# SAP/nested-hashing-psi

Measured on AMD Instinct MI355X. Metric: server PIE ciphertexts/sec, higher is better.
Workload: dtype u64

## Files before the change

nested_hashing_psi_amd/csrc/kernels.hpp:

```cpp
#pragma once
#include <hip/hip_runtime.h>

#include <atomic>
#include <vector>

#include "params.hpp"

namespace piehip {

struct PerDeviceOnce {
    std::atomic<unsigned long long> done{0};
    bool first_on_current_device()
    {
        int dev = 0;
        if (hipGetDevice(&dev) != hipSuccess || dev < 0 || dev > 63) return true;
        const unsigned long long bit = 1ULL << dev;
        return (done.fetch_or(bit) & bit) == 0;
    }
};

enum class NttKernel { radix2, blocked32, blocked16 };
struct NttRoute {
    NttKernel kernel;
    u32 s0;
// ... 7 lines not shown
    const u64 *twc = nullptr;
    const u64 *twc_fold = nullptr;
    const u64 *twk16 = nullptr;
    const DevConsts *dc;
    u32 N, logN;
    u32 num_cus;
    u32 max_slots = 0;
    bool lane_order = false;
    bool fold = false;
    NttKernel lane_kernel = NttKernel::radix2;
    u32 lane_logn = 0;
    u32 lane_T = 0;
    u32 lane_kp = 16;
    bool small_moduli = false;
    bool fold_moduli = false;
    bool xq_reuse = false;
    bool x_direct = false;
    bool fused_tensor = false;
    bool d01_eval_q = false;
    bool result_eval_q = false;
    bool digits_with_d01 = false;
    bool digit_lift_lane = false;
    bool digit_lift_std = false;
    u32 transform_cus() const
    {
        if (!max_slots) return num_cus;
        const u32 c = (max_slots + 1) / 2;
        return c < num_cus ? (c ? c : 1u) : num_cus;
    }
};
// ... 166 lines not shown
```

nested_hashing_psi_amd/csrc/kernels_ntt16.hip:

```cpp
#include <cassert>

#include "kernels.hpp"
#include "ntt16_kernel.h"

namespace piehip {

void build_twk16_table(const u64 *nat_pairs, u32 s0, u32 slice_log, std::vector<u64> &out)
{
    if (slice_log == 14)
        ntt16::build_twk_table_t<14>(nat_pairs, s0, out);
    else
        ntt16::build_twk_table_t<13>(nat_pairs, s0, out);
}

void ntt16_sigma_inverse_map(u32 logN, u32 s0, std::vector<u32> &map)
{
    const u32 N = 1u << logN, n = N >> s0;
    map.resize(N);
    for (u32 p = 0; p < N; p++) map[p] = (p / n) * n + ntt16::lane_to_std_t(p % n, n / 16);
}

template <u32 LOGNS, auto KERNEL>
static void launch_ntt16_k(const ntt16::Args &a, u32 num_cus, hipStream_t st)
{
    typedef ntt16::Geo<LOGNS> G;
    constexpr size_t lds = (size_t)G::LDS_WORDS * sizeof(u64);
    static PerDeviceOnce attr;
    if (attr.first_on_current_device()) (void)hipFuncSetAttribute((const void *)KERNEL, hipFuncAttributeMaxDynamicSharedMemorySize, (int)lds);
    const u32 slots = (LOGNS == 13 ? 2u : 1u) * num_cus;
    const u32 grid = a.nitems < slots ? a.nitems : slots;
    hipLaunchKernelGGL(KERNEL, dim3(grid), dim3(G::T), lds, st, a);
}
template <u32 LOGNS>
static void launch_ntt16_t(const ntt16::Args &a, bool inverse, bool lift, u32 num_cus, hipStream_t st, bool tensor = false, bool fd = false)
{
    using ntt16::ntt16_kernel_t;
    if (tensor && fd) launch_ntt16_k<LOGNS, ntt16_kernel_t<LOGNS, true, false, true, ArithKind::fold>>(a, num_cus, st);
    else if (tensor) launch_ntt16_k<LOGNS, ntt16_kernel_t<LOGNS, true, false, true>>(a, num_cus, st);
    else if (inverse) launch_ntt16_k<LOGNS, ntt16_kernel_t<LOGNS, true>>(a, num_cus, st);
    else if (lift) launch_ntt16_k<LOGNS, ntt16_kernel_t<LOGNS, false, true>>(a, num_cus, st);
    else launch_ntt16_k<LOGNS, ntt16_kernel_t<LOGNS, false>>(a, num_cus, st);
}

void launch_ntt16(const NttPlan &pl, u64 *data, u32 nlimbs, u32 mod_base, u32 mod_count, bool inverse, bool sigma, hipStream_t st,
                  const NttExtra *ex, const Ntt16Digits *dg)
{
    const bool folded = pl.fold;
    const u32 s0 = folded ? 1u : 0u;
    assert(ntt_route(pl, inverse, sigma, folded).kernel == NttKernel::blocked16 && (!dg || pl.digits_with_d01));
    ntt16::Args a;
    a.data = data;
    a.twp = reinterpret_cast<const ntt16::u64x2 *>(pl.twp);
    a.twk = reinterpret_cast<const ntt16::u64x2 *>(pl.twk16);
    a.dc = pl.dc;
    a.N = pl.N;
    a.s0 = s0;
    a.nitems = nlimbs << s0;
// ... 15 lines not shown
    a.lift_src = nullptr;
    a.lift_stride = 0;
    a.lift_L = 1;
    a.tsrc = nullptr;
    a.tq_L = 0;
    a.tq_first = 0;
    if (dg && !inverse) {
        a.lift_first = a.nitems;
        a.nitems += (dg->nb * dg->L * dg->L) << s0;
        a.data2 = dg->dig;
        a.lift_src = dg->d2;
        a.lift_stride = dg->stride2;
        a.lift_L = dg->L;
    }
    const bool lift = a.lift_first != ~0u;
    if (pl.lane_logn == 14)
        launch_ntt16_t<14>(a, inverse, lift, pl.transform_cus(), st);
    else
        launch_ntt16_t<13>(a, inverse, lift, pl.transform_cus(), st);
}

void launch_ntt16_tensor(const NttPlan &pl, const u64 *e, u64 *d, u32 nb, u32 M, hipStream_t st, u32 eval_q_L, bool eval_q_d2)
{
    assert(pl.fused_tensor && (!eval_q_L || ((eval_q_d2 ? pl.result_eval_q : pl.d01_eval_q) && eval_q_L < M)) && (!eval_q_d2 || eval_q_L));
    const bool folded = pl.fold;
    const u32 s0 = folded ? 1u : 0u;
    ntt16::Args a = {};
    a.data = d;
    a.twp = reinterpret_cast<const ntt16::u64x2 *>(pl.twp);
    a.twk = reinterpret_cast<const ntt16::u64x2 *>(pl.twk16);
    a.dc = pl.dc;
    a.N = pl.N;
    a.s0 = s0;
    a.tq_L = eval_q_L;
// ... 17 lines not shown
```

nested_hashing_psi_amd/csrc/ntt16_bfly.inc:

```
#define NTT16_CT1(TWC) \
    asm( \
        "v_mad_u64_u32 v[120:121], vcc, %[bl0], %[sh0], 0\n\t" \
        "v_lshl_add_u64 v[118:119], %[a0], 0, %[nq4]\n\t" \
        "v_mad_u64_u32 v[120:121], vcc, %[bh0], %[sl0], v[120:121]\n\t" \
        "v_mad_u64_u32 v[124:125], vcc, %[bl0], %[wl0], 0\n\t" \
        "v_lshlrev_b32 v117, 1, %[bh0]\n\t" \
        "v_ashrrev_i32 v122, 31, v119\n\t" \
        "v_bfi_b32 v118, v122, %[al0], v118\n\t" \
        "v_bfi_b32 v119, v122, %[ah0], v119\n\t" \
        "v_mad_u64_u32 v[126:127], vcc, %[bl0], %[wh0], 0\n\t" \
        "v_lshrrev_b64 v[120:121], 31, v[120:121]\n\t" \
        "v_mad_u64_u32 v[126:127], vcc, %[bh0], %[wl0], v[126:127]\n\t" \
        "v_mad_u64_u32 v[122:123], vcc, v117, %[sh0], v[120:121]\n\t" \
        "v_mad_u64_u32 v[124:125], vcc, v122, %[nql], v[124:125]\n\t" \
        "v_mad_u64_u32 v[126:127], vcc, v122, %[nqh], v[126:127]\n\t" \
        "v_mad_u64_u32 v[126:127], vcc, v123, %[nql], v[126:127]\n\t" \
        "v_lshl_add_u64 v[122:123], v[118:119], 0, %[q4]\n\t" \
        "v_sub_co_u32 %[bol0], vcc, v122, v124\n\t" \
        "v_add_u32 v125, v125, v126\n\t" \
        "v_lshl_add_u64 %[ao0], v[118:119], 0, v[124:125]\n\t" \
        "v_subb_co_u32 %[boh0], vcc, v123, v125, vcc\n\t" \
        : [ao0] "=v"(ao0), [bol0] "=v"(bol0), [boh0] "=v"(boh0) \
        : [a0] "v"(a0), [al0] "v"((u32)a0), [ah0] "v"((u32)(a0 >> 32)), [bl0] "v"((u32)b0), [bh0] "v"((u32)(b0 >> 32)), \
          [wl0] TWC(t0.wl), [wh0] TWC(t0.wh), [sl0] TWC(t0.sl), [sh0] TWC(t0.sh), \
// ... 120 lines not shown
        "v_mad_u64_u32 v[126:127], vcc, %[bh0], %[wl0], v[126:127]\n\t" \
        "v_mad_u64_u32 v[124:125], vcc, %[bh0], %[sh20], v[122:123]\n\t" \
        "v_mad_u64_u32 %[a0], vcc, v124, %[nql], %[a0]\n\t" \
        "v_mad_u64_u32 v[126:127], vcc, v124, %[nqh], v[126:127]\n\t" \
        "v_lshl_add_u64 v[120:121], v[120:121], 1, %[q4]\n\t" \
        "v_sub_co_u32 %[bol0], vcc, v120, %[al0]\n\t" \
        "v_mad_u64_u32 v[126:127], %[cs], v125, %[nql], v[126:127]\n\t" \
        "v_add_u32 %[ah0], %[ah0], v126\n\t" \
        "v_subb_co_u32 %[boh0], vcc, v121, %[ah0], vcc\n\t" \
        : [a0] "+v"(a0), [bol0] "=v"(bol0), [boh0] "=v"(boh0), [cs] "=s"(cs) \
        : [al0] "v"((u32)a0), [ah0] "v"((u32)(a0 >> 32)), [bl0] "v"((u32)b0), [bh0] "v"((u32)(b0 >> 32)), \
          [wl0] TWC(t0.wl), [wh0] TWC(t0.wh), [sl0] TWC(t0.sl), [sh0] TWC(t0.sh), \
          [sh20] TWC(t0.sh2), \
          [nql] "s"(m.nql), [nqh] "s"(m.nqh), [nq4] "s"(m.nq4), [q4] "s"(m.q4) \
        : "vcc", "v119", "v120", "v121", "v122", "v123", "v124", "v125", "v126", "v127")
```

nested_hashing_psi_amd/csrc/ntt16_kernel.h:

```cpp
#pragma once
#include <vector>

#include "madasm.h"
#include "params.hpp"

namespace piehip {
namespace ntt16 {

typedef u64 u64x2 __attribute__((ext_vector_type(2)));

template <u32 LOGNS>
struct Geo {
    static constexpr u32 LOGN = LOGNS;
    static constexpr u32 NS = 1u << LOGNS;
    static constexpr u32 T = NS / 16;
    static constexpr u32 W = T / 64;
    static constexpr u32 R = NS / 1024;
    static constexpr u32 LOGR = LOGNS - 10;
    static constexpr u32 CPT = 16 / R;
    static constexpr u32 LDS_WORDS = NS + NS / 16;
    static constexpr u32 TWK_PER_SLICE = W * 15 * 16 + W * 12 * 64;
};
static constexpr u32 LOGN = Geo<13>::LOGN, NS = Geo<13>::NS, T = Geo<13>::T, LDS_WORDS = Geo<13>::LDS_WORDS,
                     TWK_PER_SLICE = Geo<13>::TWK_PER_SLICE;
// ... 15 lines not shown
    u32 nql, nqh;
    u64 nq4;
    u64 q4;
};

#ifndef NTT16_CT_SEEDED
#define NTT16_CT_SEEDED 1
#endif
#define NTT16_S(x) "s"(x)
#define NTT16_V(x) "v"(x)
#include "ntt16_bfly.inc"

#ifndef NTT16_INV_H2
#define NTT16_INV_H2 1
#endif
template <bool INV, bool SC, bool H2 = SC && (!INV || NTT16_INV_H2)>
__device__ __forceinline__ void bfly(u64 &x0, u64 &y0, const Tw &t0, const ModC &m)
{
    u64 a0 = x0;
    const u64 b0 = y0;
    if (INV) {
        u32 aol0, aoh0;
        u64 bo0;
        if (SC && H2)
            NTT16_GS1H(NTT16_S);
        else if (SC)
            NTT16_GS1(NTT16_S);
        else if (H2)
            NTT16_GS1H(NTT16_V);
        else
            NTT16_GS1(NTT16_V);
        x0 = ((u64)aoh0 << 32) | aol0, y0 = bo0;
    } else {
        u32 bol0, boh0;
#if NTT16_CT_SEEDED
        u64 cs;
// ... 9 lines not shown
        x0 = a0, y0 = ((u64)boh0 << 32) | bol0;
#else
        u64 ao0;
        if (SC && H2)
            NTT16_CT1H(NTT16_S);
        else if (SC)
            NTT16_CT1(NTT16_S);
        else if (H2)
            NTT16_CT1H(NTT16_V);
        else
            NTT16_CT1(NTT16_V);
        x0 = ao0, y0 = ((u64)boh0 << 32) | bol0;
#endif
    }
}
template <bool INV, bool SC, bool H2 = SC && !INV>
__device__ __forceinline__ void bfly2(u64 &x0, u64 &y0, const Tw &t0, u64 &x1, u64 &y1, const Tw &t1, const ModC &m)
{
    bfly<INV, SC, H2>(x0, y0, t0, m);
    bfly<INV, SC, H2>(x1, y1, t1, m);
}
__device__ __forceinline__ constexpr int bfly_lo(int m, int d) { return ((m & ~(d - 1)) << 1) | (m & (d - 1)); }

typedef const __attribute__((address_space(4))) u64x2 *TwS;
typedef const __attribute__((address_space(4))) DevConsts *DcS;
__device__ __forceinline__ u64 uniform_addr(const void *p)
{
    const u64 v = (u64)p;
    const u32 lo = __builtin_amdgcn_readfirstlane((u32)v), hi = __builtin_amdgcn_readfirstlane((u32)(v >> 32));
    return ((u64)hi << 32) | lo;
}

__device__ __forceinline__ u64 csub_neg(u64 x, u64 negm)
{
    u32 lo, hi;
    asm("v_lshl_add_u64 v[126:127], %[x], 0, %[nm]\n\t"
        "v_ashrrev_i32 v125, 31, v127\n\t"
        "v_bfi_b32 %[lo], v125, %[xl], v126\n\t"
        "v_bfi_b32 %[hi], v125, %[xh], v127"
        : [lo] "=&v"(lo), [hi] "=&v"(hi)
        : [x] "v"(x), [xl] "v"((u32)x), [xh] "v"((u32)(x >> 32)), [nm] "s"(negm)
        : "v125", "v126", "v127");
    return ((u64)hi << 32) | lo;
}

__device__ __forceinline__ const u64 *at_bytes(const u64 *ubase, u32 boff)
{
    return reinterpret_cast<const u64 *>(reinterpret_cast<const char *>(ubase) + boff);
}
__device__ __forceinline__ u64 *at_bytes(u64 *ubase, u32 boff) { return reinterpret_cast<u64 *>(reinterpret_cast<char *>(ubase) + boff); }
__device__ __forceinline__ const u64x2 *at_bytes(const u64x2 *ubase, u32 boff)
{
    return reinterpret_cast<const u64x2 *>(reinterpret_cast<const char *>(ubase) + boff);
}

template <u32 CPT>
__device__ __forceinline__ void row_get(u64 *x, int r, const u64 *p)
// ... 241 lines not shown
                const u64 fc = csub2_neg(k ? vc[j].y : vc[j].x, nq4, nq2);
                const u64 fd = csub2_neg(k ? vd[j].y : vd[j].x, nq4, nq2);
                colacc_mac(c, split30(fc), split30(fd));
            }
            x[2 * j + k] = FD ? colacc_fold_to_4q(c.c0, c.c1, c.c2, nq) : colacc123_to_4q(c.c0, c.c1, c.c2, mu, nq);
        }
        NTT16_FENCE();
        if (j + DEPTH < 8) NTT16_TLOAD(j + DEPTH);
    }
#undef NTT16_TLOAD
}

template <u32 LOGNS, bool INV, bool LIFT = false, bool TENSOR = false, ArithKind KIND = ArithKind::barrett>
__global__ void __launch_bounds__(Geo<LOGNS>::T, 4) ntt16_kernel_t(Args a)
{
    static_assert(KIND == ArithKind::barrett || (TENSOR && KIND == ArithKind::fold), "the kind: of the tensor load phase, column accumulators");
    constexpr bool FD = KIND == ArithKind::fold;
    typedef Geo<LOGNS> G;
    constexpr u32 NS = G::NS, T = G::T, R = G::R, LOGR = G::LOGR, CPT = G::CPT, TWK_PER_SLICE = G::TWK_PER_SLICE;
    extern __shared__ __attribute__((aligned(16))) u64 lds[];
    const u32 tau = threadIdx.x;
    const u32 w = __builtin_amdgcn_readfirstlane(tau >> 6), l = tau & 63;
    const u32 la = l >> 2, lc = l & 3;
    u64 *const p1 = lds + phi(CPT * tau);
    u64 *const p2 = lds + phi(1024 * w + l);
    u64 *const p3 = lds + 1088 * w + 68 * la + lc;
    u64 *const p4 = lds + phi(1024 * w + 16 * l);

    u64 x[16];
    auto limb_of = [&](u32 it) -> u32 {
        u32 lb = it >> a.s0;
        if (!INV && a.skip_L) {
// ... 87 lines not shown
                };
                if (a.s0 == 1) {
                    u64x2 fw;
                    fw.x = dcs->fold_w[lj];
                    fw.y = dcs->fold_w_sh[lj] >> 1;
                    const Tw t = make_tw(fw);
                    u64 y[16];
#pragma unroll
                    for (int r = 0; r < (int)R; r++) {
                        row_get_global<CPT>(x, r, at_bytes(src + 1024 * r, coffb));
                        row_get_global<CPT>(y, r, at_bytes(src + NS + 1024 * r, coffb));
                    }
#pragma unroll
                    for (int k = 0; k < 16; k++) {
                        u64 u0 = lift1(x[k]), v0 = lift1(y[k]);
                        bfly<false, true>(u0, v0, t, mc);
                        x[k] = blk ? v0 : u0;
                    }
                } else {
#pragma unroll
                    for (int r = 0; r < (int)R; r++) row_get_global<CPT>(x, r, at_bytes(src + 1024 * r, coffb));
#pragma unroll
                    for (int k = 0; k < 16; k++) x[k] = lift1(x[k]);
                }
            } else {
#pragma unroll
                for (int r = 0; r < (int)R; r++) row_get_global<CPT>(x, r, at_bytes(g + 1024 * r, coffb));
            }
            NTT16_PRIO_F(1);
#pragma unroll
            for (int s = 0; s < (int)LOGR; s++) {
                const int d = (int)(R >> 1) >> s;
#pragma unroll
                for (int r = 0; r < (int)R; r++) {
                    if (r & d) continue;
                    const Tw t = make_tw(NTT16_TWL(1u << s, (u32)r >> (LOGR - s)));
#pragma unroll
                    for (int c = 0; c < (int)CPT; c++) bfly<false, true>(x[CPT * r + c], x[CPT * (r + d) + c], t, mc);
                }
            }
            NTT16_STAMP(1);
            __syncthreads();
            NTT16_STAMP(2);
#pragma unroll
            for (int r = 0; r < (int)R; r++) row_put<CPT>(x, r, p1 + 1088 * r);
            NTT16_STAMP(3);
            __syncthreads();
            NTT16_STAMP(4);
            NTT16_PRIO_F(2);
#pragma unroll
            for (int k = 0; k < 16; k++) x[k] = p2[68 * k];
#pragma unroll
            for (int sb = 0; sb < 4; sb++) {
                const int d = 8 >> sb;
#pragma unroll
                for (int mm = 0; mm < 8; mm += 2) {
                    const int k0 = bfly_lo(mm, d), k1 = bfly_lo(mm + 1, d);
                    const Tw t0 = make_tw(NTT16_TWL(G::W << sb, (w << sb) + ((u32)k0 >> (4 - sb))));
                    const Tw t1 = make_tw(NTT16_TWL(G::W << sb, (w << sb) + ((u32)k1 >> (4 - sb))));
                    bfly2<false, true>(x[k0], x[k0 + d], t0, x[k1], x[k1 + d], t1, mc);
                }
            }
            NTT16_LOAD3(t7, 0);
            NTT16_LOAD3(t8, 1);
#pragma unroll
            for (int k = 0; k < 16; k++) p2[68 * k] = x[k];
            NTT16_STAMP(5);
            wave_sync();
            NTT16_PRIO_F(3);
#pragma unroll
            for (int k = 0; k < 16; k++) x[k] = p3[4 * k + 2 * (k >> 3)];
            NTT16_LOAD3(t9, 2);
            NTT16_FENCE();
            {
                const Tw t = make_tw(t7[0]);
#pragma unroll
                for (int k = 0; k < 8; k += 2) bfly2<false, false, true>(x[k], x[k + 8], t, x[k + 1], x[k + 9], t, mc);
            }
            NTT16_LOAD3H(t10, 3, 0);
            NTT16_FENCE();
#pragma unroll
            for (int mm = 0; mm < 8; mm += 2) {
                const int k0 = bfly_lo(mm, 4), k1 = bfly_lo(mm + 1, 4);
                bfly2<false, false, true>(x[k0], x[k0 + 4], make_tw(t8[k0 >> 3]), x[k1], x[k1 + 4], make_tw(t8[k1 >> 3]), mc);
            }
            NTT16_LOAD3H(t10, 3, 4);
            NTT16_FENCE();
#pragma unroll
            for (int mm = 0; mm < 8; mm += 2) {
                const int k0 = bfly_lo(mm, 2), k1 = bfly_lo(mm + 1, 2);
                bfly2<false, false>(x[k0], x[k0 + 2], make_tw(t9[k0 >> 2]), x[k1], x[k1 + 2], make_tw(t9[k1 >> 2]), mc);
            }
            NTT16_LOAD4(t11, 0, 4);
            NTT16_FENCE();
#pragma unroll
            for (int k = 0; k < 16; k += 4)
                bfly2<false, false>(x[k], x[k + 1], make_tw(t10[k >> 1]), x[k + 2], x[k + 3], make_tw(t10[(k >> 1) + 1]), mc);
#pragma unroll
            for (int k = 0; k < 16; k++) p3[4 * k + 2 * (k >> 3)] = x[k];
            NTT16_STAMP(6);
            wave_sync();
            NTT16_PRIO_F(4);
#pragma unroll
            for (int j = 0; j < 8; j++) {
                const u64x2 v = *reinterpret_cast<const u64x2 *>(p4 + 2 * j);
                x[2 * j] = v.x;
                x[2 * j + 1] = v.y;
            }
            NTT16_LOAD4(t12, 4, 4);
            NTT16_FENCE();
#pragma unroll
            for (int g4 = 0; g4 < 4; g4++) {
                const Tw t = make_tw(t11[g4]);
                bfly2<false, false>(x[4 * g4], x[4 * g4 + 2], t, x[4 * g4 + 1], x[4 * g4 + 3], t, mc);
                if (g4 == 1) {
                    NTT16_FENCE();
                    _Pragma("unroll") for (int j_ = 4; j_ < 8; j_++) t12[j_] = *at_bytes(tw4 + 64 * (4 + j_), lb);
                    NTT16_FENCE();
                }
            }
            NTT16_FENCE();
#pragma unroll
            for (int k = 0; k < 16; k += 4)
                bfly2<false, false>(x[k], x[k + 1], make_tw(t12[k >> 1]), x[k + 2], x[k + 3], make_tw(t12[(k >> 1) + 1]), mc);
            NTT16_STAMP(7);
            const bool lazy = (a.flags & F_LAZY_OUT) != 0 && !lift;
            if (!lazy) {
#pragma unroll
                for (int k = 0; k < 16; k++) x[k] = csub_neg(csub_neg(csub_neg(x[k], 0 - q4), 0 - q2), 0 - q);
            }
#pragma unroll
            for (int j = 0; j < 8; j++) {
                u64x2 v;
                v.x = x[2 * j], v.y = x[2 * j + 1];
                pair_put_global(v, at_bytes(g + 2 * T * j, voffb));
            }
            NTT16_STAMP(8);
        } else {
            NTT16_STAMP(0);
            NTT16_PRIO_I(0);
            NTT16_LOAD4(t12, 4, 4);
            const bool is_x = !TENSOR && (a.flags & F_STD_IN) && a.copy_out && (limb / (2 * a.copy_L)) % a.copy_K == 0;
            u64 *co = nullptr;
            if (is_x) {
// ... 46 lines not shown
                else
                    tensor_load<T, false, FD>(x, pa, pb, pc, pd, voffb, q, mu);
            } else {
                const u64 *src = x_in ? co : g;
                asm("" : "+s"(src));
#pragma unroll
                for (int j = 0; j < 8; j++) {
                    const u64x2 v = pair_get_global(at_bytes(src + 2 * T * j, voffb));
                    x[2 * j] = v.x, x[2 * j + 1] = v.y;
                }
            }
            NTT16_FENCE();
            _Pragma("unroll") for (int j_ = 4; j_ < 8; j_++) t12[j_] = *at_bytes(tw4 + 64 * (4 + j_), lb);
            NTT16_FENCE();
            NTT16_PRIO_I(1);
#pragma unroll
            for (int k = 0; k < 16; k += 4) {
                bfly2<true, false>(x[k], x[k + 1], make_tw(t12[k >> 1]), x[k + 2], x[k + 3], make_tw(t12[(k >> 1) + 1]), mc);
                if (k == 4) {
                    NTT16_FENCE();
                    NTT16_LOAD4(t11, 0, 4);
                    NTT16_FENCE();
                }
            }
            NTT16_LOAD3(t10, 3);
            NTT16_FENCE();
#pragma unroll
            for (int g4 = 0; g4 < 4; g4++) {
                const Tw t = make_tw(t11[g4]);
                bfly2<true, false>(x[4 * g4], x[4 * g4 + 2], t, x[4 * g4 + 1], x[4 * g4 + 3], t, mc);
            }
            NTT16_STAMP(1);
            NTT16_STAMP(2);
#pragma unroll
            for (int j = 0; j < 8; j++) {
                u64x2 v;
                v.x = x[2 * j];
                v.y = x[2 * j + 1];
                *reinterpret_cast<u64x2 *>(p4 + 2 * j) = v;
            }
            wave_sync();
            NTT16_STAMP(3);
            NTT16_PRIO_I(2);
#pragma unroll
            for (int k = 0; k < 16; k++) x[k] = p3[4 * k + 2 * (k >> 3)];
            NTT16_LOAD3(t9, 2);
            NTT16_FENCE();
#pragma unroll
            for (int k = 0; k < 16; k += 4)
                bfly2<true, false>(x[k], x[k + 1], make_tw(t10[k >> 1]), x[k + 2], x[k + 3], make_tw(t10[(k >> 1) + 1]), mc);
            NTT16_LOAD3(t8, 1);
            NTT16_LOAD3(t7, 0);
            NTT16_FENCE();
#pragma unroll
            for (int mm = 0; mm < 8; mm += 2) {
                const int k0 = bfly_lo(mm, 2), k1 = bfly_lo(mm + 1, 2);
                bfly2<true, false>(x[k0], x[k0 + 2], make_tw(t9[k0 >> 2]), x[k1], x[k1 + 2], make_tw(t9[k1 >> 2]), mc);
            }
            NTT16_FENCE();
#pragma unroll
            for (int mm = 0; mm < 8; mm += 2) {
                const int k0 = bfly_lo(mm, 4), k1 = bfly_lo(mm + 1, 4);
                bfly2<true, false>(x[k0], x[k0 + 4], make_tw(t8[k0 >> 3]), x[k1], x[k1 + 4], make_tw(t8[k1 >> 3]), mc);
            }
            {
                const Tw t = make_tw(t7[0]);
#pragma unroll
                for (int k = 0; k < 8; k += 2) bfly2<true, false>(x[k], x[k + 8], t, x[k + 1], x[k + 9], t, mc);
            }
#pragma unroll
            for (int k = 0; k < 16; k++) p3[4 * k + 2 * (k >> 3)] = x[k];
            wave_sync();
            NTT16_STAMP(4);
            NTT16_PRIO_I(3);
#pragma unroll
            for (int k = 0; k < 16; k++) x[k] = p2[68 * k];
#pragma unroll
            for (int sb = 3; sb >= 0; sb--) {
                const int d = 8 >> sb;
#pragma unroll
                for (int mm = 0; mm < 8; mm += 2) {
                    const int k0 = bfly_lo(mm, d), k1 = bfly_lo(mm + 1, d);
                    const Tw t0 = make_tw(NTT16_TWL(G::W << sb, (w << sb) + ((u32)k0 >> (4 - sb))));
                    const Tw t1 = make_tw(NTT16_TWL(G::W << sb, (w << sb) + ((u32)k1 >> (4 - sb))));
                    bfly2<true, true>(x[k0], x[k0 + d], t0, x[k1], x[k1 + d], t1, mc);
                }
            }
#pragma unroll
            for (int k = 0; k < 16; k++) p2[68 * k] = x[k];
            NTT16_STAMP(5);
            __syncthreads();
            NTT16_STAMP(6);
            NTT16_PRIO_I(4);
#pragma unroll
            for (int r = 0; r < (int)R; r++) row_get<CPT>(x, r, p1 + 1088 * r);
            __syncthreads();
#pragma unroll
            for (int s = (int)LOGR - 1; s >= 0; s--) {
                const int d = (int)(R >> 1) >> s;
#pragma unroll
                for (int r = 0; r < (int)R; r++) {
                    if (r & d) continue;
                    const Tw t = make_tw(NTT16_TWL(1u << s, (u32)r >> (LOGR - s)));
#pragma unroll
                    for (int c = 0; c < (int)CPT; c++) bfly<true, true>(x[CPT * r + c], x[CPT * (r + d) + c], t, mc);
                }
            }
            NTT16_STAMP(7);
            const u64 n_inv = dcs->mod[mod].n_inv, n_inv_sh = dcs->mod[mod].n_inv_sh;
            if (!(a.flags & F_FOLDED)) {
#pragma unroll
                for (int k = 0; k < 16; k++) {
                    if (a.s0 == 0)
                        x[k] = csub_neg(mul_shoup_lazy(x[k], n_inv, n_inv_sh, q), 0 - q);
                    else
                        x[k] = csub_neg(csub_neg(x[k], 0 - q2), 0 - q);
                }
            }
#pragma unroll
            for (int r = 0; r < (int)R; r++) row_put_global<CPT>(x, r, at_bytes(g + 1024 * r, coffb));
            NTT16_STAMP(8);
// ... 12 lines not shown
```

nested_hashing_psi_amd/csrc/piehip.cpp:

```cpp
#include "piehip_ctx.hpp"

#include <random>

using namespace piehip;

static thread_local std::string g_err;
static const char *KNAMES[PIEHIP_NKERNELS] = {"stage_a_mac", "ntt_fwd", "ntt_inv",  "expand",   "tensor",    "scale_round",
                                              "digits",      "relin",   "mask_mul", "encode",   "automorph", "other",
                                              "event_pair",  "tensor_ntt_inv", "result_ntt_inv", "limb_drop", "result_ntt_fwd",
                                              "deg2_finish"};
static void free_workspace(piehip_ctx *h);

namespace piehip {

int fail(int code, const std::string &msg)
{
    g_err = msg;
    return code;
}

void join_pending(piehip_ctx *h)
{
    if (!h->pending_join) return;
    for (size_t g = 0; g < h->ev_join.size(); g++) (void)hipStreamWaitEvent(h->stream, h->ev_join[g], 0);
// ... 128 lines not shown
    do {                                                                               \
        hipError_t e_ = (expr);                                                        \
        if (e_ != hipSuccess) return std::string(#expr) + ": " + hipGetErrorString(e_); \
    } while (0)
    const u32 N = hp.N, M = hp.M, logN = hp.logN;
    pl.N = N;
    pl.logN = logN;
    {
        bool lazy_ok = true, small_moduli = true, fold_moduli = true;
        for (u32 a = 0; a <= M; a++) {
            if (hp.moduli[a] >> 60) lazy_ok = false;
            if (a < M && (hp.moduli[a] >> 59) != 1) small_moduli = false;
            if (a < M && (1ull << 60) - hp.moduli[a] >= COLACC_FOLD_MAX_D) fold_moduli = false;
        }
        ntt_plan_decide(pl, lazy_ok, small_moduli, fold_moduli);
        hipDeviceProp_t prop;
        pl.num_cus = (hipGetDeviceProperties(&prop, h->device) == hipSuccess && prop.multiProcessorCount > 0) ? (u32)prop.multiProcessorCount : 256u;
    }
    TBL_(upload_table(h, &hp.dc, 1, d_dc));
    pl.dc = *d_dc;
    {
        std::vector<u64> pairs((size_t)(M + 1) * 4 * N);
        u64 *tables = nullptr;
        TBL_(upload_table(h, (const u64 *)nullptr, pairs.size(), &tables));
        pl.tables = tables;
        for (u32 a = 0; a <= M; a++) {
            for (const std::vector<u64> *t : {&hp.tw[a], &hp.tw_sh[a], &hp.itw[a], &hp.itw_sh[a]}) {
                TBL_(hipMemcpy(tables, t->data(), sizeof(u64) * N, hipMemcpyHostToDevice));
                tables += N;
            }
// ... 1044 lines not shown
```

Baseline: 81200.

## Use fold-reduction butterflies in blocked16 NTT for pseudo-Mersenne moduli

Result: faster. 83500 (median of 6 runs) (+2.8%).

```diff
diff --git a/nested_hashing_psi_amd/csrc/kernels.hpp b/nested_hashing_psi_amd/csrc/kernels.hpp
--- a/nested_hashing_psi_amd/csrc/kernels.hpp
+++ b/nested_hashing_psi_amd/csrc/kernels.hpp
@@ -45,6 +45,7 @@
     u32 lane_kp = 16;
     bool small_moduli = false;
     bool fold_moduli = false;
+    u32 fold_mod_count = 0;
     bool xq_reuse = false;
     bool x_direct = false;
     bool fused_tensor = false;
diff --git a/nested_hashing_psi_amd/csrc/kernels_ntt16.hip b/nested_hashing_psi_amd/csrc/kernels_ntt16.hip
--- a/nested_hashing_psi_amd/csrc/kernels_ntt16.hip
+++ b/nested_hashing_psi_amd/csrc/kernels_ntt16.hip
@@ -31,16 +31,26 @@
     const u32 grid = a.nitems < slots ? a.nitems : slots;
     hipLaunchKernelGGL(KERNEL, dim3(grid), dim3(G::T), lds, st, a);
 }
+template <u32 LOGNS, ArithKind KIND>
+static void launch_ntt16_kind(const ntt16::Args &a, bool inverse, bool lift, u32 num_cus, hipStream_t st, bool tensor)
+{
+    using ntt16::ntt16_kernel_t;
+    if (tensor) launch_ntt16_k<LOGNS, ntt16_kernel_t<LOGNS, true, false, true, KIND>>(a, num_cus, st);
+    else if (inverse) launch_ntt16_k<LOGNS, ntt16_kernel_t<LOGNS, true, false, false, KIND>>(a, num_cus, st);
+    else if (lift) launch_ntt16_k<LOGNS, ntt16_kernel_t<LOGNS, false, true, false, KIND>>(a, num_cus, st);
+    else launch_ntt16_k<LOGNS, ntt16_kernel_t<LOGNS, false, false, false, KIND>>(a, num_cus, st);
+}
 template <u32 LOGNS>
 static void launch_ntt16_t(const ntt16::Args &a, bool inverse, bool lift, u32 num_cus, hipStream_t st, bool tensor = false, bool fd = false)
 {
-    using ntt16::ntt16_kernel_t;
-    if (tensor && fd) launch_ntt16_k<LOGNS, ntt16_kernel_t<LOGNS, true, false, true, ArithKind::fold>>(a, num_cus, st);
-    else if (tensor) launch_ntt16_k<LOGNS, ntt16_kernel_t<LOGNS, true, false, true>>(a, num_cus, st);
-    else if (inverse) launch_ntt16_k<LOGNS, ntt16_kernel_t<LOGNS, true>>(a, num_cus, st);
-    else if (lift) launch_ntt16_k<LOGNS, ntt16_kernel_t<LOGNS, false, true>>(a, num_cus, st);
-    else launch_ntt16_k<LOGNS, ntt16_kernel_t<LOGNS, false>>(a, num_cus, st);
+#if NTT16_FOLD_BFLY
+    if (fd) return launch_ntt16_kind<LOGNS, ArithKind::fold>(a, inverse, lift, num_cus, st, tensor);
+#else
+    if (fd && tensor) return launch_ntt16_k<LOGNS, ntt16::ntt16_kernel_t<LOGNS, true, false, true, ArithKind::fold>>(a, num_cus, st);
+#endif
+    launch_ntt16_kind<LOGNS, ArithKind::barrett>(a, inverse, lift, num_cus, st, tensor);
 }
+static bool launch_folds(const NttPlan &pl, u32 mod_base, u32 mod_count) { return pl.fold_moduli && mod_base + mod_count <= pl.fold_mod_count; }
 
 void launch_ntt16(const NttPlan &pl, u64 *data, u32 nlimbs, u32 mod_base, u32 mod_count, bool inverse, bool sigma, hipStream_t st,
                   const NttExtra *ex, const Ntt16Digits *dg)
@@ -86,10 +96,11 @@
         a.lift_L = dg->L;
     }
     const bool lift = a.lift_first != ~0u;
+    const bool fd = launch_folds(pl, mod_base, mod_count) && (!dg || dg->L <= pl.fold_mod_count);
     if (pl.lane_logn == 14)
-        launch_ntt16_t<14>(a, inverse, lift, pl.transform_cus(), st);
+        launch_ntt16_t<14>(a, inverse, lift, pl.transform_cus(), st, false, fd);
     else
-        launch_ntt16_t<13>(a, inverse, lift, pl.transform_cus(), st);
+        launch_ntt16_t<13>(a, inverse, lift, pl.transform_cus(), st, false, fd);
 }
 
 void launch_ntt16_tensor(const NttPlan &pl, const u64 *e, u64 *d, u32 nb, u32 M, hipStream_t st, u32 eval_q_L, bool eval_q_d2)
diff --git a/nested_hashing_psi_amd/csrc/ntt16_bfly.inc b/nested_hashing_psi_amd/csrc/ntt16_bfly.inc
--- a/nested_hashing_psi_amd/csrc/ntt16_bfly.inc
+++ b/nested_hashing_psi_amd/csrc/ntt16_bfly.inc
@@ -158,3 +158,151 @@
           [sh20] TWC(t0.sh2), \
           [nql] "s"(m.nql), [nqh] "s"(m.nqh), [nq4] "s"(m.nq4), [q4] "s"(m.q4) \
         : "vcc", "v119", "v120", "v121", "v122", "v123", "v124", "v125", "v126", "v127")
+#define NTT16_CTF1(TWC) \
+    asm( \
+        "v_lshrrev_b32 v124, 28, %[ah0]\n\t" \
+        "v_and_b32 %[ah0], 0xfffffff, %[ah0]\n\t" \
+        "v_lshlrev_b32 v119, 1, %[bh0]\n\t" \
+        "v_mad_u64_u32 v[122:123], vcc, %[bl0], %[sh0], 0\n\t" \
+        "v_mad_u64_u32 %[a0], vcc, v124, %[nql], %[a0]\n\t" \
+        "v_mad_u64_u32 v[122:123], vcc, %[bh0], %[sl0], v[122:123]\n\t" \
+        "v_mad_u64_u32 v[126:127], vcc, %[bl0], %[wh0], 0\n\t" \
+        "v_lshl_add_u64 v[120:121], %[a0], 1, %[q4]\n\t" \
+        "v_mad_u64_u32 %[a0], vcc, %[bl0], %[wl0], %[a0]\n\t" \
+        "v_lshrrev_b64 v[122:123], 31, v[122:123]\n\t" \
+        "v_mad_u64_u32 v[126:127], vcc, %[bh0], %[wl0], v[126:127]\n\t" \
+        "v_mad_u64_u32 v[124:125], vcc, v119, %[sh0], v[122:123]\n\t" \
+        "v_mad_u64_u32 %[a0], vcc, v124, %[nql], %[a0]\n\t" \
+        "v_mad_u64_u32 v[126:127], vcc, v124, %[nqh], v[126:127]\n\t" \
+        "v_sub_co_u32 %[bol0], vcc, v120, %[al0]\n\t" \
+        "v_mad_u64_u32 v[126:127], %[cs], v125, %[nql], v[126:127]\n\t" \
+        "v_add_u32 %[ah0], %[ah0], v126\n\t" \
+        "v_subb_co_u32 %[boh0], vcc, v121, %[ah0], vcc\n\t" \
+        : [a0] "+v"(a0), [bol0] "=v"(bol0), [boh0] "=v"(boh0), [cs] "=s"(cs) \
+        : [al0] "v"((u32)a0), [ah0] "v"((u32)(a0 >> 32)), [bl0] "v"((u32)b0), [bh0] "v"((u32)(b0 >> 32)), \
+          [wl0] TWC(t0.wl), [wh0] TWC(t0.wh), [sl0] TWC(t0.sl), [sh0] TWC(t0.sh), \
+          [nql] "s"(m.nql), [nqh] "s"(m.nqh), [q4] "s"(m.q4) \
+        : "vcc", "v119", "v120", "v121", "v122", "v123", "v124", "v125", "v126", "v127")
+#define NTT16_CTF1H(TWC) \
+    asm( \
+        "v_lshrrev_b32 v124, 28, %[ah0]\n\t" \
+        "v_and_b32 %[ah0], 0xfffffff, %[ah0]\n\t" \
+        "v_mad_u64_u32 v[122:123], vcc, %[bl0], %[sh0], 0\n\t" \
+        "v_mad_u64_u32 %[a0], vcc, v124, %[nql], %[a0]\n\t" \
+        "v_mad_u64_u32 v[122:123], vcc, %[bh0], %[sl0], v[122:123]\n\t" \
+        "v_mad_u64_u32 v[126:127], vcc, %[bl0], %[wh0], 0\n\t" \
+        "v_lshl_add_u64 v[120:121], %[a0], 1, %[q4]\n\t" \
+        "v_mad_u64_u32 %[a0], vcc, %[bl0], %[wl0], %[a0]\n\t" \
+        "v_lshrrev_b64 v[122:123], 31, v[122:123]\n\t" \
+        "v_mad_u64_u32 v[126:127], vcc, %[bh0], %[wl0], v[126:127]\n\t" \
+        "v_mad_u64_u32 v[124:125], vcc, %[bh0], %[sh20], v[122:123]\n\t" \
+        "v_mad_u64_u32 %[a0], vcc, v124, %[nql], %[a0]\n\t" \
+        "v_mad_u64_u32 v[126:127], vcc, v124, %[nqh], v[126:127]\n\t" \
+        "v_sub_co_u32 %[bol0], vcc, v120, %[al0]\n\t" \
+        "v_mad_u64_u32 v[126:127], %[cs], v125, %[nql], v[126:127]\n\t" \
+        "v_add_u32 %[ah0], %[ah0], v126\n\t" \
+        "v_subb_co_u32 %[boh0], vcc, v121, %[ah0], vcc\n\t" \
+        : [a0] "+v"(a0), [bol0] "=v"(bol0), [boh0] "=v"(boh0), [cs] "=s"(cs) \
+        : [al0] "v"((u32)a0), [ah0] "v"((u32)(a0 >> 32)), [bl0] "v"((u32)b0), [bh0] "v"((u32)(b0 >> 32)), \
+          [wl0] TWC(t0.wl), [wh0] TWC(t0.wh), [sl0] TWC(t0.sl), [sh0] TWC(t0.sh), \
+          [sh20] TWC(t0.sh2), \
+          [nql] "s"(m.nql), [nqh] "s"(m.nqh), [q4] "s"(m.q4) \
+        : "vcc", "v119", "v120", "v121", "v122", "v123", "v124", "v125", "v126", "v127")
+#define NTT16_GSF1(TWC) \
+    asm( \
+        "v_lshl_add_u64 v[122:123], %[a0], 0, %[q4]\n\t" \
+        "v_lshl_add_u64 v[124:125], %[a0], 0, %[b0]\n\t" \
+        "v_sub_co_u32 v118, vcc, v122, %[bl0]\n\t" \
+        "v_lshrrev_b32 v117, 28, v125\n\t" \
+        "v_and_b32 v125, 0xfffffff, v125\n\t" \
+        "v_subb_co_u32 v119, vcc, v123, %[bh0], vcc\n\t" \
+        "v_mad_u64_u32 %[ao0], vcc, v117, %[nql], v[124:125]\n\t" \
+        "v_mad_u64_u32 v[124:125], vcc, v118, %[wl0], 0\n\t" \
+        "v_mad_u64_u32 v[126:127], vcc, v118, %[wh0], 0\n\t" \
+        "v_mad_u64_u32 v[120:121], vcc, v118, %[sh0], 0\n\t" \
+        "v_mad_u64_u32 v[120:121], vcc, v119, %[sl0], v[120:121]\n\t" \
+        "v_mad_u64_u32 v[126:127], vcc, v119, %[wl0], v[126:127]\n\t" \
+        "v_lshlrev_b32 v117, 1, v119\n\t" \
+        "v_lshrrev_b64 v[120:121], 31, v[120:121]\n\t" \
+        "v_mad_u64_u32 v[122:123], vcc, v117, %[sh0], v[120:121]\n\t" \
+        "v_mad_u64_u32 v[126:127], vcc, v122, %[nqh], v[126:127]\n\t" \
+        "v_mad_u64_u32 v[126:127], vcc, v123, %[nql], v[126:127]\n\t" \
+        "v_add_u32 v125, v125, v126\n\t" \
+        "v_mad_u64_u32 %[bo0], vcc, v122, %[nql], v[124:125]\n\t" \
+        : [ao0] "=&v"(ao0), [bo0] "=v"(bo0) \
+        : [a0] "v"(a0), [b0] "v"(b0), [bl0] "v"((u32)b0), [bh0] "v"((u32)(b0 >> 32)), \
+          [wl0] TWC(t0.wl), [wh0] TWC(t0.wh), [sl0] TWC(t0.sl), [sh0] TWC(t0.sh), \
+          [nql] "s"(m.nql), [nqh] "s"(m.nqh), [q4] "s"(m.q4) \
+        : "vcc", "v117", "v118", "v119", "v120", "v121", "v122", "v123", "v124", "v125", "v126", "v127")
+#define NTT16_GSF1H(TWC) \
+    asm( \
+        "v_lshl_add_u64 v[122:123], %[a0], 0, %[q4]\n\t" \
+        "v_lshl_add_u64 v[124:125], %[a0], 0, %[b0]\n\t" \
+        "v_sub_co_u32 v118, vcc, v122, %[bl0]\n\t" \
+        "v_lshrrev_b32 v117, 28, v125\n\t" \
+        "v_and_b32 v125, 0xfffffff, v125\n\t" \
+        "v_subb_co_u32 v119, vcc, v123, %[bh0], vcc\n\t" \
+        "v_mad_u64_u32 %[ao0], vcc, v117, %[nql], v[124:125]\n\t" \
+        "v_mad_u64_u32 v[124:125], vcc, v118, %[wl0], 0\n\t" \
+        "v_mad_u64_u32 v[126:127], vcc, v118, %[wh0], 0\n\t" \
+        "v_mad_u64_u32 v[120:121], vcc, v118, %[sh0], 0\n\t" \
+        "v_mad_u64_u32 v[120:121], vcc, v119, %[sl0], v[120:121]\n\t" \
+        "v_mad_u64_u32 v[126:127], vcc, v119, %[wl0], v[126:127]\n\t" \
+        "v_lshrrev_b64 v[120:121], 31, v[120:121]\n\t" \
+        "v_mad_u64_u32 v[122:123], vcc, v119, %[sh20], v[120:121]\n\t" \
+        "v_mad_u64_u32 v[126:127], vcc, v122, %[nqh], v[126:127]\n\t" \
+        "v_mad_u64_u32 v[126:127], vcc, v123, %[nql], v[126:127]\n\t" \
+        "v_add_u32 v125, v125, v126\n\t" \
+        "v_mad_u64_u32 %[bo0], vcc, v122, %[nql], v[124:125]\n\t" \
+        : [ao0] "=&v"(ao0), [bo0] "=v"(bo0) \
+        : [a0] "v"(a0), [b0] "v"(b0), [bl0] "v"((u32)b0), [bh0] "v"((u32)(b0 >> 32)), \
+          [wl0] TWC(t0.wl), [wh0] TWC(t0.wh), [sl0] TWC(t0.sl), [sh0] TWC(t0.sh), \
+          [sh20] TWC(t0.sh2), \
+          [nql] "s"(m.nql), [nqh] "s"(m.nqh), [q4] "s"(m.q4) \
+        : "vcc", "v117", "v118", "v119", "v120", "v121", "v122", "v123", "v124", "v125", "v126", "v127")
+#define NTT16_GSN1(TWC) \
+    asm( \
+        "v_lshl_add_u64 v[122:123], %[a0], 0, %[q4]\n\t" \
+        "v_sub_co_u32 v118, vcc, v122, %[bl0]\n\t" \
+        "v_lshl_add_u64 %[ao0], %[a0], 0, %[b0]\n\t" \
+        "v_mad_u64_u32 v[124:125], %[cs], v118, %[wl0], 0\n\t" \
+        "v_subb_co_u32 v119, vcc, v123, %[bh0], vcc\n\t" \
+        "v_mad_u64_u32 v[126:127], vcc, v118, %[wh0], 0\n\t" \
+        "v_mad_u64_u32 v[120:121], vcc, v118, %[sh0], 0\n\t" \
+        "v_mad_u64_u32 v[120:121], vcc, v119, %[sl0], v[120:121]\n\t" \
+        "v_mad_u64_u32 v[126:127], vcc, v119, %[wl0], v[126:127]\n\t" \
+        "v_lshlrev_b32 v117, 1, v119\n\t" \
+        "v_lshrrev_b64 v[120:121], 31, v[120:121]\n\t" \
+        "v_mad_u64_u32 v[122:123], vcc, v117, %[sh0], v[120:121]\n\t" \
+        "v_mad_u64_u32 v[126:127], vcc, v122, %[nqh], v[126:127]\n\t" \
+        "v_mad_u64_u32 v[126:127], vcc, v123, %[nql], v[126:127]\n\t" \
+        "v_add_u32 v125, v125, v126\n\t" \
+        "v_mad_u64_u32 %[bo0], vcc, v122, %[nql], v[124:125]\n\t" \
+        : [ao0] "=&v"(ao0), [bo0] "=v"(bo0), [cs] "=&s"(cs) \
+        : [a0] "v"(a0), [b0] "v"(b0), [bl0] "v"((u32)b0), [bh0] "v"((u32)(b0 >> 32)), \
+          [wl0] TWC(t0.wl), [wh0] TWC(t0.wh), [sl0] TWC(t0.sl), [sh0] TWC(t0.sh), \
+          [nql] "s"(m.nql), [nqh] "s"(m.nqh), [q4] "s"(m.q4) \
+        : "vcc", "v117", "v118", "v119", "v120", "v121", "v122", "v123", "v124", "v125", "v126", "v127")
+#define NTT16_GSN1H(TWC) \
+    asm( \
+        "v_lshl_add_u64 v[122:123], %[a0], 0, %[q4]\n\t" \
+        "v_sub_co_u32 v118, vcc, v122, %[bl0]\n\t" \
+        "v_lshl_add_u64 %[ao0], %[a0], 0, %[b0]\n\t" \
+        "v_mad_u64_u32 v[124:125], %[cs], v118, %[wl0], 0\n\t" \
+        "v_subb_co_u32 v119, vcc, v123, %[bh0], vcc\n\t" \
+        "v_mad_u64_u32 v[126:127], vcc, v118, %[wh0], 0\n\t" \
+        "v_mad_u64_u32 v[120:121], vcc, v118, %[sh0], 0\n\t" \
+        "v_mad_u64_u32 v[120:121], vcc, v119, %[sl0], v[120:121]\n\t" \
+        "v_mad_u64_u32 v[126:127], vcc, v119, %[wl0], v[126:127]\n\t" \
+        "v_lshrrev_b64 v[120:121], 31, v[120:121]\n\t" \
+        "v_mad_u64_u32 v[122:123], vcc, v119, %[sh20], v[120:121]\n\t" \
+        "v_mad_u64_u32 v[126:127], vcc, v122, %[nqh], v[126:127]\n\t" \
+        "v_mad_u64_u32 v[126:127], vcc, v123, %[nql], v[126:127]\n\t" \
+        "v_add_u32 v125, v125, v126\n\t" \
+        "v_mad_u64_u32 %[bo0], vcc, v122, %[nql], v[124:125]\n\t" \
+        : [ao0] "=&v"(ao0), [bo0] "=v"(bo0), [cs] "=&s"(cs) \
+        : [a0] "v"(a0), [b0] "v"(b0), [bl0] "v"((u32)b0), [bh0] "v"((u32)(b0 >> 32)), \
+          [wl0] TWC(t0.wl), [wh0] TWC(t0.wh), [sl0] TWC(t0.sl), [sh0] TWC(t0.sh), \
+          [sh20] TWC(t0.sh2), \
+          [nql] "s"(m.nql), [nqh] "s"(m.nqh), [q4] "s"(m.q4) \
+        : "vcc", "v117", "v118", "v119", "v120", "v121", "v122", "v123", "v124", "v125", "v126", "v127")
diff --git a/nested_hashing_psi_amd/csrc/ntt16_kernel.h b/nested_hashing_psi_amd/csrc/ntt16_kernel.h
--- a/nested_hashing_psi_amd/csrc/ntt16_kernel.h
+++ b/nested_hashing_psi_amd/csrc/ntt16_kernel.h
@@ -53,12 +53,52 @@
 #ifndef NTT16_INV_H2
 #define NTT16_INV_H2 1
 #endif
-template <bool INV, bool SC, bool H2 = SC && (!INV || NTT16_INV_H2)>
-__device__ __forceinline__ void bfly(u64 &x0, u64 &y0, const Tw &t0, const ModC &m)
+#ifndef NTT16_FOLD_BFLY
+#define NTT16_FOLD_BFLY 1
+#endif
+template <bool INV, bool SC, bool H2 = SC && (!INV || NTT16_INV_H2), ArithKind KIND = ArithKind::barrett>
+__device__ __forceinline__ void bfly(u64 &x0, u64 &y0, const Tw &t0, const ModC &m, bool below_T = false)
 {
     u64 a0 = x0;
     const u64 b0 = y0;
-    if (INV) {
+    if (INV && KIND == ArithKind::fold && NTT16_FOLD_BFLY) {
+        u64 ao0, bo0;
+        if (below_T) {
+            u64 cs;
+            if (SC && H2)
+                NTT16_GSN1H(NTT16_S);
+            else if (SC)
+                NTT16_GSN1(NTT16_S);
+            else if (H2)
+                NTT16_GSN1H(NTT16_V);
+            else
+                NTT16_GSN1(NTT16_V);
+            (void)cs;
+        } else {
+            if (SC && H2)
+                NTT16_GSF1H(NTT16_S);
+            else if (SC)
+                NTT16_GSF1(NTT16_S);
+            else if (H2)
+                NTT16_GSF1H(NTT16_V);
+            else
+                NTT16_GSF1(NTT16_V);
+        }
+        x0 = ao0, y0 = bo0;
+    } else if (!INV && KIND == ArithKind::fold && NTT16_FOLD_BFLY) {
+        u32 bol0, boh0;
+        u64 cs;
+        if (SC && H2)
+            NTT16_CTF1H(NTT16_S);
+        else if (SC)
+            NTT16_CTF1(NTT16_S);
+        else if (H2)
+            NTT16_CTF1H(NTT16_V);
+        else
+            NTT16_CTF1(NTT16_V);
+        (void)cs;
+        x0 = a0, y0 = ((u64)boh0 << 32) | bol0;
+    } else if (INV) {
         u32 aol0, aoh0;
         u64 bo0;
         if (SC && H2)
@@ -98,12 +138,24 @@
 #endif
     }
 }
-template <bool INV, bool SC, bool H2 = SC && !INV>
-__device__ __forceinline__ void bfly2(u64 &x0, u64 &y0, const Tw &t0, u64 &x1, u64 &y1, const Tw &t1, const ModC &m)
-{
-    bfly<INV, SC, H2>(x0, y0, t0, m);
-    bfly<INV, SC, H2>(x1, y1, t1, m);
-}
+template <bool INV, bool SC, bool H2 = SC && !INV, ArithKind KIND = ArithKind::barrett>
+__device__ __forceinline__ void bfly2(u64 &x0, u64 &y0, const Tw &t0, u64 &x1, u64 &y1, const Tw &t1, const ModC &m, bool below_T0 = false,
+                                      bool below_T1 = false)
+{
+    bfly<INV, SC, H2, KIND>(x0, y0, t0, m, below_T0);
+    bfly<INV, SC, H2, KIND>(x1, y1, t1, m, below_T1);
+}
+struct GsRanges {
+    u32 below_T = 0;
+    __device__ __forceinline__ constexpr bool nofold(int k, int d) const { return ((below_T >> k) & (below_T >> (k + d)) & 1u) != 0; }
+    __device__ __forceinline__ constexpr void stage(int d)
+    {
+        u32 n = 0;
+        for (int k = 0; k < 16; k++)
+            if (!(k & d) && !nofold(k, d)) n |= 1u << k;
+        below_T = n;
+    }
+};
 __device__ __forceinline__ constexpr int bfly_lo(int m, int d) { return ((m & ~(d - 1)) << 1) | (m & (d - 1)); }
 
 typedef const __attribute__((address_space(4))) u64x2 *TwS;
@@ -125,6 +177,23 @@
         : [lo] "=&v"(lo), [hi] "=&v"(hi)
         : [x] "v"(x), [xl] "v"((u32)x), [xh] "v"((u32)(x >> 32)), [nm] "s"(negm)
         : "v125", "v126", "v127");
+    return ((u64)hi << 32) | lo;
+}
+
+__device__ __forceinline__ u64 fold_csub_neg(u64 x, u64 negq)
+{
+    u32 lo, hi;
+    asm("v_lshrrev_b32 v125, 28, %[xh]\n\t"
+        "v_and_b32 v124, 0xf0000000, %[xh]\n\t"
+        "v_mad_u64_u32 v[126:127], vcc, v125, %[d], %[x]\n\t"
+        "v_sub_u32 v127, v127, v124\n\t"
+        "v_lshl_add_u64 v[124:125], v[126:127], 0, %[nq]\n\t"
+        "v_ashrrev_i32 v123, 31, v125\n\t"
+        "v_bfi_b32 %[lo], v123, v126, v124\n\t"
+        "v_bfi_b32 %[hi], v123, v127, v125"
+        : [lo] "=&v"(lo), [hi] "=&v"(hi)
+        : [x] "v"(x), [xh] "v"((u32)(x >> 32)), [nq] "s"(negq), [d] "s"((u32)negq)
+        : "vcc", "v123", "v124", "v125", "v126", "v127");
     return ((u64)hi << 32) | lo;
 }
 
@@ -396,8 +465,9 @@
 template <u32 LOGNS, bool INV, bool LIFT = false, bool TENSOR = false, ArithKind KIND = ArithKind::barrett>
 __global__ void __launch_bounds__(Geo<LOGNS>::T, 4) ntt16_kernel_t(Args a)
 {
-    static_assert(KIND == ArithKind::barrett || (TENSOR && KIND == ArithKind::fold), "the kind: of the tensor load phase, column accumulators");
+    static_assert(KIND == ArithKind::barrett || (KIND == ArithKind::fold && (TENSOR || NTT16_FOLD_BFLY)), "the kinds of 60-bit moduli");
     constexpr bool FD = KIND == ArithKind::fold;
+    constexpr ArithKind BK = NTT16_FOLD_BFLY ? KIND : ArithKind::barrett;
     typedef Geo<LOGNS> G;
     constexpr u32 NS = G::NS, T = G::T, R = G::R, LOGR = G::LOGR, CPT = G::CPT, TWK_PER_SLICE = G::TWK_PER_SLICE;
     extern __shared__ __attribute__((aligned(16))) u64 lds[];
@@ -515,7 +585,7 @@
 #pragma unroll
                     for (int k = 0; k < 16; k++) {
                         u64 u0 = lift1(x[k]), v0 = lift1(y[k]);
-                        bfly<false, true>(u0, v0, t, mc);
+                        bfly<false, true, true, BK>(u0, v0, t, mc);
                         x[k] = blk ? v0 : u0;
                     }
                 } else {
@@ -537,7 +607,7 @@
                     if (r & d) continue;
                     const Tw t = make_tw(NTT16_TWL(1u << s, (u32)r >> (LOGR - s)));
 #pragma unroll
-                    for (int c = 0; c < (int)CPT; c++) bfly<false, true>(x[CPT * r + c], x[CPT * (r + d) + c], t, mc);
+                    for (int c = 0; c < (int)CPT; c++) bfly<false, true, true, BK>(x[CPT * r + c], x[CPT * (r + d) + c], t, mc);
                 }
             }
             NTT16_STAMP(1);
@@ -559,7 +629,7 @@
                     const int k0 = bfly_lo(mm, d), k1 = bfly_lo(mm + 1, d);
                     const Tw t0 = make_tw(NTT16_TWL(G::W << sb, (w << sb) + ((u32)k0 >> (4 - sb))));
                     const Tw t1 = make_tw(NTT16_TWL(G::W << sb, (w << sb) + ((u32)k1 >> (4 - sb))));
-                    bfly2<false, true>(x[k0], x[k0 + d], t0, x[k1], x[k1 + d], t1, mc);
+                    bfly2<false, true, true, BK>(x[k0], x[k0 + d], t0, x[k1], x[k1 + d], t1, mc);
                 }
             }
             NTT16_LOAD3(t7, 0);
@@ -576,27 +646,27 @@
             {
                 const Tw t = make_tw(t7[0]);
 #pragma unroll
-                for (int k = 0; k < 8; k += 2) bfly2<false, false, true>(x[k], x[k + 8], t, x[k + 1], x[k + 9], t, mc);
+                for (int k = 0; k < 8; k += 2) bfly2<false, false, true, BK>(x[k], x[k + 8], t, x[k + 1], x[k + 9], t, mc);
             }
             NTT16_LOAD3H(t10, 3, 0);
             NTT16_FENCE();
 #pragma unroll
             for (int mm = 0; mm < 8; mm += 2) {
                 const int k0 = bfly_lo(mm, 4), k1 = bfly_lo(mm + 1, 4);
-                bfly2<false, false, true>(x[k0], x[k0 + 4], make_tw(t8[k0 >> 3]), x[k1], x[k1 + 4], make_tw(t8[k1 >> 3]), mc);
+                bfly2<false, false, true, BK>(x[k0], x[k0 + 4], make_tw(t8[k0 >> 3]), x[k1], x[k1 + 4], make_tw(t8[k1 >> 3]), mc);
             }
             NTT16_LOAD3H(t10, 3, 4);
             NTT16_FENCE();
 #pragma unroll
             for (int mm = 0; mm < 8; mm += 2) {
                 const int k0 = bfly_lo(mm, 2), k1 = bfly_lo(mm + 1, 2);
-                bfly2<false, false>(x[k0], x[k0 + 2], make_tw(t9[k0 >> 2]), x[k1], x[k1 + 2], make_tw(t9[k1 >> 2]), mc);
+                bfly2<false, false, false, BK>(x[k0], x[k0 + 2], make_tw(t9[k0 >> 2]), x[k1], x[k1 + 2], make_tw(t9[k1 >> 2]), mc);
             }
             NTT16_LOAD4(t11, 0, 4);
             NTT16_FENCE();
 #pragma unroll
             for (int k = 0; k < 16; k += 4)
-                bfly2<false, false>(x[k], x[k + 1], make_tw(t10[k >> 1]), x[k + 2], x[k + 3], make_tw(t10[(k >> 1) + 1]), mc);
+                bfly2<false, false, false, BK>(x[k], x[k + 1], make_tw(t10[k >> 1]), x[k + 2], x[k + 3], make_tw(t10[(k >> 1) + 1]), mc);
 #pragma unroll
             for (int k = 0; k < 16; k++) p3[4 * k + 2 * (k >> 3)] = x[k];
             NTT16_STAMP(6);
@@ -613,7 +683,7 @@
 #pragma unroll
             for (int g4 = 0; g4 < 4; g4++) {
                 const Tw t = make_tw(t11[g4]);
-                bfly2<false, false>(x[4 * g4], x[4 * g4 + 2], t, x[4 * g4 + 1], x[4 * g4 + 3], t, mc);
+                bfly2<false, false, false, BK>(x[4 * g4], x[4 * g4 + 2], t, x[4 * g4 + 1], x[4 * g4 + 3], t, mc);
                 if (g4 == 1) {
                     NTT16_FENCE();
                     _Pragma("unroll") for (int j_ = 4; j_ < 8; j_++) t12[j_] = *at_bytes(tw4 + 64 * (4 + j_), lb);
@@ -623,12 +693,13 @@
             NTT16_FENCE();
 #pragma unroll
             for (int k = 0; k < 16; k += 4)
-                bfly2<false, false>(x[k], x[k + 1], make_tw(t12[k >> 1]), x[k + 2], x[k + 3], make_tw(t12[(k >> 1) + 1]), mc);
+                bfly2<false, false, false, BK>(x[k], x[k + 1], make_tw(t12[k >> 1]), x[k + 2], x[k + 3], make_tw(t12[(k >> 1) + 1]), mc);
             NTT16_STAMP(7);
             const bool lazy = (a.flags & F_LAZY_OUT) != 0 && !lift;
             if (!lazy) {
 #pragma unroll
-                for (int k = 0; k < 16; k++) x[k] = csub_neg(csub_neg(csub_neg(x[k], 0 - q4), 0 - q2), 0 - q);
+                for (int k = 0; k < 16; k++)
+                    x[k] = BK == ArithKind::fold ? fold_csub_neg(x[k], 0 - q) : csub_neg(csub_neg(csub_neg(x[k], 0 - q4), 0 - q2), 0 - q);
             }
 #pragma unroll
             for (int j = 0; j < 8; j++) {
@@ -705,9 +776,11 @@
             _Pragma("unroll") for (int j_ = 4; j_ < 8; j_++) t12[j_] = *at_bytes(tw4 + 64 * (4 + j_), lb);
             NTT16_FENCE();
             NTT16_PRIO_I(1);
+            GsRanges rs;
 #pragma unroll
             for (int k = 0; k < 16; k += 4) {
-                bfly2<true, false>(x[k], x[k + 1], make_tw(t12[k >> 1]), x[k + 2], x[k + 3], make_tw(t12[(k >> 1) + 1]), mc);
+                bfly2<true, false, false, BK>(x[k], x[k + 1], make_tw(t12[k >> 1]), x[k + 2], x[k + 3], make_tw(t12[(k >> 1) + 1]), mc,
+                                              rs.nofold(k, 1), rs.nofold(k + 2, 1));
                 if (k == 4) {
                     NTT16_FENCE();
                     NTT16_LOAD4(t11, 0, 4);
@@ -716,10 +789,12 @@
             }
             NTT16_LOAD3(t10, 3);
             NTT16_FENCE();
+            rs.stage(1);
 #pragma unroll
             for (int g4 = 0; g4 < 4; g4++) {
                 const Tw t = make_tw(t11[g4]);
-                bfly2<true, false>(x[4 * g4], x[4 * g4 + 2], t, x[4 * g4 + 1], x[4 * g4 + 3], t, mc);
+                bfly2<true, false, false, BK>(x[4 * g4], x[4 * g4 + 2], t, x[4 * g4 + 1], x[4 * g4 + 3], t, mc, rs.nofold(4 * g4, 2),
+                                              rs.nofold(4 * g4 + 1, 2));
             }
             NTT16_STAMP(1);
             NTT16_STAMP(2);
@@ -737,27 +812,35 @@
             for (int k = 0; k < 16; k++) x[k] = p3[4 * k + 2 * (k >> 3)];
             NTT16_LOAD3(t9, 2);
             NTT16_FENCE();
+            rs = GsRanges();
 #pragma unroll
             for (int k = 0; k < 16; k += 4)
-                bfly2<true, false>(x[k], x[k + 1], make_tw(t10[k >> 1]), x[k + 2], x[k + 3], make_tw(t10[(k >> 1) + 1]), mc);
+                bfly2<true, false, false, BK>(x[k], x[k + 1], make_tw(t10[k >> 1]), x[k + 2], x[k + 3], make_tw(t10[(k >> 1) + 1]), mc,
+                                              rs.nofold(k, 1), rs.nofold(k + 2, 1));
             NTT16_LOAD3(t8, 1);
             NTT16_LOAD3(t7, 0);
             NTT16_FENCE();
+            rs.stage(1);
 #pragma unroll
             for (int mm = 0; mm < 8; mm += 2) {
                 const int k0 = bfly_lo(mm, 2), k1 = bfly_lo(mm + 1, 2);
-                bfly2<true, false>(x[k0], x[k0 + 2], make_tw(t9[k0 >> 2]), x[k1], x[k1 + 2], make_tw(t9[k1 >> 2]), mc);
-            }
-            NTT16_FENCE();
+                bfly2<true, false, false, BK>(x[k0], x[k0 + 2], make_tw(t9[k0 >> 2]), x[k1], x[k1 + 2], make_tw(t9[k1 >> 2]), mc, rs.nofold(k0, 2),
+                                              rs.nofold(k1, 2));
+            }
+            NTT16_FENCE();
+            rs.stage(2);
 #pragma unroll
             for (int mm = 0; mm < 8; mm += 2) {
                 const int k0 = bfly_lo(mm, 4), k1 = bfly_lo(mm + 1, 4);
-                bfly2<true, false>(x[k0], x[k0 + 4], make_tw(t8[k0 >> 3]), x[k1], x[k1 + 4], make_tw(t8[k1 >> 3]), mc);
-            }
+                bfly2<true, false, false, BK>(x[k0], x[k0 + 4], make_tw(t8[k0 >> 3]), x[k1], x[k1 + 4], make_tw(t8[k1 >> 3]), mc, rs.nofold(k0, 4),
+                                              rs.nofold(k1, 4));
+            }
+            rs.stage(4);
             {
                 const Tw t = make_tw(t7[0]);
 #pragma unroll
-                for (int k = 0; k < 8; k += 2) bfly2<true, false>(x[k], x[k + 8], t, x[k + 1], x[k + 9], t, mc);
+                for (int k = 0; k < 8; k += 2)
+                    bfly2<true, false, false, BK>(x[k], x[k + 8], t, x[k + 1], x[k + 9], t, mc, rs.nofold(k, 8), rs.nofold(k + 1, 8));
             }
 #pragma unroll
             for (int k = 0; k < 16; k++) p3[4 * k + 2 * (k >> 3)] = x[k];
@@ -766,6 +849,7 @@
             NTT16_PRIO_I(3);
 #pragma unroll
             for (int k = 0; k < 16; k++) x[k] = p2[68 * k];
+            rs = GsRanges();
 #pragma unroll
             for (int sb = 3; sb >= 0; sb--) {
                 const int d = 8 >> sb;
@@ -774,8 +858,9 @@
                     const int k0 = bfly_lo(mm, d), k1 = bfly_lo(mm + 1, d);
                     const Tw t0 = make_tw(NTT16_TWL(G::W << sb, (w << sb) + ((u32)k0 >> (4 - sb))));
                     const Tw t1 = make_tw(NTT16_TWL(G::W << sb, (w << sb) + ((u32)k1 >> (4 - sb))));
-                    bfly2<true, true>(x[k0], x[k0 + d], t0, x[k1], x[k1 + d], t1, mc);
-                }
+                    bfly2<true, true, false, BK>(x[k0], x[k0 + d], t0, x[k1], x[k1 + d], t1, mc, rs.nofold(k0, d), rs.nofold(k1, d));
+                }
+                rs.stage(d);
             }
 #pragma unroll
             for (int k = 0; k < 16; k++) p2[68 * k] = x[k];
@@ -786,6 +871,7 @@
 #pragma unroll
             for (int r = 0; r < (int)R; r++) row_get<CPT>(x, r, p1 + 1088 * r);
             __syncthreads();
+            rs = GsRanges();
 #pragma unroll
             for (int s = (int)LOGR - 1; s >= 0; s--) {
                 const int d = (int)(R >> 1) >> s;
@@ -794,8 +880,10 @@
                     if (r & d) continue;
                     const Tw t = make_tw(NTT16_TWL(1u << s, (u32)r >> (LOGR - s)));
 #pragma unroll
-                    for (int c = 0; c < (int)CPT; c++) bfly<true, true>(x[CPT * r + c], x[CPT * (r + d) + c], t, mc);
-                }
+                    for (int c = 0; c < (int)CPT; c++)
+                        bfly<true, true, NTT16_INV_H2 != 0, BK>(x[CPT * r + c], x[CPT * (r + d) + c], t, mc, rs.nofold(CPT * r + c, CPT * d));
+                }
+                rs.stage(CPT * d);
             }
             NTT16_STAMP(7);
             const u64 n_inv = dcs->mod[mod].n_inv, n_inv_sh = dcs->mod[mod].n_inv_sh;
diff --git a/nested_hashing_psi_amd/csrc/piehip.cpp b/nested_hashing_psi_amd/csrc/piehip.cpp
--- a/nested_hashing_psi_amd/csrc/piehip.cpp
+++ b/nested_hashing_psi_amd/csrc/piehip.cpp
@@ -166,6 +166,7 @@
             if (a < M && (1ull << 60) - hp.moduli[a] >= COLACC_FOLD_MAX_D) fold_moduli = false;
         }
         ntt_plan_decide(pl, lazy_ok, small_moduli, fold_moduli);
+        pl.fold_mod_count = pl.fold_moduli ? M : 0;
         hipDeviceProp_t prop;
         pl.num_cus = (hipGetDeviceProperties(&prop, h->device) == hipSuccess && prop.multiProcessorCount > 0) ? (u32)prop.multiProcessorCount : 256u;
     }
```
